# Tencent/FeatherCNN

Measured on AMD Instinct MI355X. Metric: images/sec fp32 forward @224x224, higher is better.
Workload: dtype f32; 1 GPU; vgg16 whole net (40 layers in the model file, 20 after fusion level 3), batch 32 per GPU, 224x224x3, fp32, synthetic ...; net=vgg16, mode=net, per_gpu_batch=32, global_batch=32, parallelism=batch-shard x1, launch=hipGraph replay per step, conv_routing=fhip_conv_select_algo_tuned

## Files before the change

__graft_entry__.py:

```python
from __future__ import annotations

import os
import subprocess
import sys

ROOT = os.path.dirname(os.path.abspath(__file__))
if ROOT not in sys.path:
    sys.path.insert(0, ROOT)


def build() -> None:
    jobs = str(min(8, os.cpu_count() or 1))
    subprocess.run(["make", "-s", "-j", jobs, "-C", os.path.join(ROOT, "feathercnn_amd", "csrc")], check=True)
    subprocess.run(["make", "-s", "-C", os.path.join(ROOT, "oracle"), "port"], check=True)
    subprocess.run(["make", "-s", "-C", os.path.join(ROOT, "oracle"), "ref"], check=True)
    import feathercnn_amd
    feathercnn_amd.load_library()
    from feathercnn_amd import _lib
    _lib.load_gconv_library()
    _lib.load_deconv_library()
    _lib.load_inorm_library()
    _lib.load_shuffle_library()
    _lib.load_canvas_library()
    _lib.load_atrous_library()
    _lib.load_gate_library()
    from feathercnn_amd import provenance
    provenance.write_stamp()


def smoke() -> None:
    import numpy as np
    import torch

    import oracle
    from feathercnn_amd import ConvLayer, ConvParam
    from oracle import conv_geom, nerr, synth

    if not torch.cuda.is_available():
        raise RuntimeError("smoke() needs a GPU")
    if not os.path.exists(os.path.join(ROOT, "feathercnn_amd", "libfeather_hip.so")):
# ... 123 lines not shown
    print(f"smoke tiny_dilated ({sum(a == 'ATROUS' for _, _, a in net.layers())} dilated layers): normalised error = {e:.2e}")
    if not (e <= 1e-4):
        raise AssertionError(f"smoke tiny_dilated: parity failed ({e})")
    import gate_ref
    p, b, i, o = model_zoo.tiny_se()
    x = np.random.default_rng(11).uniform(-1, 1, (2, 3, 24, 24)).astype(np.float32)
    net = Net(fusion=2)
    net.LoadParam(p)
    net.LoadWeights(b)
    net.FeedInput(i, x)
    net.Forward()
    e = gate_ref.nerr(net.Extract(o), gate_ref.Net(p, b).run(i, x, o))
    print(f"smoke tiny_se ({sum(a == 'GATE' and t == 'Pooling' for t, _, a in net.layers())} collapsed SE blocks): normalised error = {e:.2e}")
    if not (e <= 1e-4):
        raise AssertionError(f"smoke tiny_se: parity failed ({e})")
    print("smoke OK")


if __name__ == "__main__":
    build()
    if len(sys.argv) > 1 and sys.argv[1] == "smoke":
        smoke()
```

feathercnn_amd/_lib.py:

```python
from __future__ import annotations

import ctypes
import os

_HERE = os.path.dirname(os.path.abspath(__file__))
_LOADED = {}

STAGE_NAMES = ("wino_input", "wino_gemm", "wino_output", "igemm", "depthwise", "init", "wino_chain")


class fhip_conv_param(ctypes.Structure):
    _fields_ = [(n, ctypes.c_int) for n in (
        "output_channels", "input_channels", "input_h", "input_w", "kernel_h", "kernel_w", "output_h", "output_w",
        "stride_h", "stride_w", "pad_left", "pad_bottom", "pad_right", "pad_top", "group", "bias_term", "activation")]


class fhip_winograd_plan(ctypes.Structure):
    _fields_ = [("tiles_x", ctypes.c_int), ("tiles_y", ctypes.c_int), ("tiles_per_image", ctypes.c_int),
                ("columns", ctypes.c_int), ("columns_padded", ctypes.c_int), ("column_block", ctypes.c_int), ("frequency_points", ctypes.c_int), ("tile_outputs", ctypes.c_int),
                ("in_channels_padded", ctypes.c_int),
                ("out_channels_padded", ctypes.c_int), ("v_offset_bytes", ctypes.c_size_t), ("v_bytes", ctypes.c_size_t),
                ("m_offset_bytes", ctypes.c_size_t), ("m_bytes", ctypes.c_size_t), ("u_bytes", ctypes.c_size_t)]


# ... 23 lines not shown
    "fhip_conv_init": (_I, [_P, _I, _V, _V, _V]),
    "fhip_conv_forward": (_I, [_P, _I, _I, _V, _V, _V, _V, _V, _V]),
    "fhip_winograd_f63_plan": (_I, [_P, _I, ctypes.POINTER(fhip_winograd_plan)]),
    "fhip_winograd_f63_plan_canvas": (_I, [_P, _I, _I, ctypes.POINTER(fhip_winograd_plan)]),
    "fhip_winograd_f63_canvas_param": (_I, [_P, _I, _P]),
    "fhip_winograd_f63_transform_kernel": (_I, [_P, _V, _V, _V]),
    "fhip_winograd_f63_input_transform": (_I, [_P, _I, _V, _V, _V]),
    "fhip_winograd_f63_tile_gemm": (_I, [_P, _I, _V, _V, _V, _V]),
    "fhip_winograd_f63_output_transform": (_I, [_P, _I, _V, _V, _V, _V]),
    "fhip_stage_timing_enable": (_I, [_I]),
    "fhip_stage_timing_collect": (_I, [ctypes.POINTER(ctypes.c_double), ctypes.POINTER(ctypes.c_longlong)]),
    "fhip_last_error": (ctypes.c_char_p, []),
    "fhip_version": (ctypes.c_char_p, []),
    "fhip_device_info": (_I, [ctypes.c_char_p, _I, ctypes.POINTER(_I), ctypes.POINTER(_I)]),
    "fhip_conv_streams_1x1": (_I, [_P, _I, _I]),
    "fhip_calibrate_mfma_f32": (_I, [ctypes.POINTER(ctypes.c_double), ctypes.POINTER(ctypes.c_double), _V]),
    "fhip_relu": (_I, [_V, _V, _SZ, _V]),
    "fhip_add": (_I, [_V, _V, _V, _SZ, _I, _V]),
    "fhip_affine": (_I, [_V, _V, _V, _V, _I, _I, _I, _I, _V]),
    "fhip_conv_can_fuse_residual": (_I, [_P, _I]),
    "fhip_conv_forward_residual": (_I, [_P, _I, _I, _V, _V, _V, _V, _V, _V, _V]),
    "fhip_conv_can_fuse_dw_pw": (_I, [_P, _P, _I]),
    "fhip_conv_forward_dw_pw": (_I, [_P, _P, _I, _V, _V, _V, _V, _V, _V, _V]),
    "fhip_conv_can_chain_winograd": (_I, [_P, _I, _P, _I, _I]),
    "fhip_conv_forward_chained": (_I, [_P, _I, _V, _V, _V, _V, _V, _V, _P, _V, _I, _V]),
    "fhip_winograd_f63_output_to_next_input": (_I, [_P, _P, _I, _V, _V, _V, _I, _V]),
    "fhip_conv_can_fuse_siblings": (_I, [_P, _I, _P, _I, _I]),
    "fhip_conv_siblings_geometry": (_I, [_P, _P, _P]),
    "fhip_conv_forward_siblings": (_I, [_P, _P, _I, _V, _V, _V, _V, _V, _V]),
    "fhip_conv_can_fuse_first_winograd": (_I, [_P, _P, _I, _I]),
# ... 23 lines not shown
    "fhip_net_load_weights_mem": (_I, [_V, _V, _SZ]),
    "fhip_net_load_weights_device": (_I, [_V, _V, _SZ]),
    "fhip_net_feed_input": (_I, [_V, ctypes.c_char_p, _I, _I, _I, _I, _V, _I]),
    "fhip_net_feed_pixels": (_I, [_V, ctypes.c_char_p, _I, _V, _I, _I, _I, _I, _I, _V, _V, _I]),
    "fhip_net_feed_yuv420sp": (_I, [_V, ctypes.c_char_p, _I, _V, _I, _I, _I, _I, _I, _I, _V, _V, _I]),
    "fhip_net_feed_pixel_images": (_I, [_V, ctypes.c_char_p, _I, _V, _I, _I, _I, _V, _V, _I]),
    "fhip_net_forward": (_I, [_V]),
    "fhip_net_extract": (_I, [_V, ctypes.c_char_p, ctypes.POINTER(_V), _PI, _PI, _PI, _PI]),
    "fhip_net_extract_host": (_I, [_V, ctypes.c_char_p, _V, _SZ]),
    "fhip_net_layer_count": (_I, [_V]),
    "fhip_net_layer_info": (_I, [_V, _I, ctypes.c_char_p, ctypes.c_char_p, _I, _PI]),
    "fhip_net_layer_conv_param": (_I, [_V, _I, _P, _PI]),
    "fhip_net_layer_fused_pointwise": (_I, [_V, _I, _P, _PI]),
    "fhip_net_layer_chain": (_I, [_V, _I, _PI, _PI]),
    "fhip_net_layer_canvas": (_I, [_V, _I, _PI]),
    "fhip_net_layer_sibling": (_I, [_V, _I, _PI]),
    "fhip_net_layer_residual": (_I, [_V, _I, _PI]),
    "fhip_net_forward_timed": (_I, [_V, ctypes.POINTER(ctypes.c_float)]),
    "fhip_net_memory": (_I, [_V, ctypes.POINTER(_SZ), ctypes.POINTER(_SZ), ctypes.POINTER(_SZ)]),
}

PIXOUT_SIGNATURES = {
    "fhip_pixout_channels": (_I, [_I]),
    "fhip_float_to_pixels": (_I, [_V, _SZ, _V, _I, _I, _I, _I, _I, _I, _V, _V, _V]),
    "fhip_float_to_pixels_host": (_I, [_V, _SZ, _V, _I, _I, _I, _I, _I, _I, _V, _V, _V]),
    "fhip_pixout_last_error": (ctypes.c_char_p, []),
}

GCONV_SIGNATURES = {
    "fhip_gconv_supported": (_I, [_P]),
# ... 70 lines not shown
    "fhip_atrous_get_buffer_size_route": (_I, [_AP, _I, ctypes.c_char_p, ctypes.POINTER(_SZ), ctypes.POINTER(_SZ)]),
    "fhip_atrous_init_route": (_I, [_AP, _V, _V, _V, ctypes.c_char_p]),
    "fhip_atrous_forward_route": (_I, [_AP, _I, _V, _V, _V, _V, _V, _V, ctypes.c_char_p]),
    "fhip_atrous_last_error": (ctypes.c_char_p, []),
}

GATE_SIGNATURES = {
    "fhip_channel_gate_forward": (_I, [_I, _I, _I, _I, _V, _V, _V, _V, _I, _V]),
    "fhip_squeeze_get_buffer_size": (_I, [_I, _I, _I, _I, ctypes.POINTER(_SZ)]),
    "fhip_squeeze_forward": (_I, [_I, _I, _I, _I, _V, _V, _V, _V]),
    "fhip_excite_forward": (_I, [_I, _I, _I, _V, _V, _V, _V, _V, _V, _I, _I, _FL, _FL, _V]),
    "fhip_excite_forward_slices": (_I, [_I, _I, _I, _I, _V, _V, _V, _V, _V, _V, _I, _I, _FL, _FL, _V]),
    "fhip_gate_activation_forward": (_I, [_I, _V, _V, _I, _I, _I, _FL, _FL, _V]),
    "fhip_gate_route": (_I, [_I, _I, _I, _I, _I, _V, _V, _V, ctypes.c_char_p, _I]),
    "fhip_gate_last_error": (ctypes.c_char_p, []),
}


def _load(path, signatures):
    lib = _LOADED.get(path)
    if lib is None:
        import torch
        if not os.path.exists(path):
            raise RuntimeError(f"feathercnn_amd: HIP library {path} is missing -- run `python -c 'import __graft_entry__ as g; "
                               "g.build()'` (or `make -C feathercnn_amd/csrc`). There is no CPU fallback.")
        lib = ctypes.CDLL(path)
        for name, (res, args) in signatures.items():
            fn = getattr(lib, name)
            fn.restype = res
            fn.argtypes = args
# ... 59 lines not shown

def atrous_path() -> str:
    return os.path.join(_HERE, "libfeather_atrous.so")


def load_atrous_library():
    return _load(atrous_path(), ATROUS_SIGNATURES)


def gate_path() -> str:
    return os.path.join(_HERE, "libfeather_gate.so")


def load_gate_library():
    return _load(gate_path(), GATE_SIGNATURES)
```

feathercnn_amd/csrc/capi.hip:

```cpp
#include <string.h>
#include <stdlib.h>

#include <algorithm>
#include <mutex>
#include <string>
#include <vector>

#include "common.h"
#include "feather_hip/feather_net.h"

namespace fhip
{
int winograd_plan(const fhip_conv_param& p, int batch, fhip_winograd_plan* plan);
int winograd_transform_kernel(const fhip_conv_param& p, float* u, const float* kernel, hipStream_t s);
int winograd_input_transform(const fhip_conv_param& p, int batch, float* v, const float* input, hipStream_t s);
int winograd_tile_gemm(const fhip_conv_param& p, int batch, float* m, const float* u, const float* v, hipStream_t s);
int winograd_output_transform(const fhip_conv_param& p, int batch, float* output, const float* m, const float* bias,
                              hipStream_t s, int pool = 0);
bool winograd_can_pool(const fhip_conv_param& p);
bool winograd_can_chain(const fhip_conv_param& p, const fhip_conv_param& next, int pool);
bool winograd_can_fuse_first(const fhip_conv_param& first, const fhip_conv_param& next, int batch);
fhip_conv_param igemm_twin_geometry(const fhip_conv_param& a, const fhip_conv_param& b);
bool igemm_twin_applicable(const fhip_conv_param& a, const fhip_conv_param& b, int batch);
int igemm_twin_forward(const fhip_conv_param& a, const fhip_conv_param& b, int batch, float* out_a, float* out_b, const float* in, const float* packed,
                       const float* bias, hipStream_t s);
int winograd_input_from_first(const fhip_conv_param& first, const fhip_conv_param& next, int batch, float* v, const float* input,
                              const float* first_kernel, const float* first_bias, hipStream_t s);
int winograd_output_to_next_input(const fhip_conv_param& p, const fhip_conv_param& next, int batch, float* vn, const float* m, const float* bias,
                                  hipStream_t s, int pool);
void igemm_packed_dims(const fhip_conv_param& p, int* kd_padded, int* k_padded);
int igemm_init(const fhip_conv_param& p, float* packed, const float* kernel, hipStream_t s);
int igemm_forward(const fhip_conv_param& p, int batch, float* out, const float* in, const float* packed, const float* bias,
                  float* buffer, bool force_no_act, hipStream_t s, const float* residual = nullptr);
size_t igemm_buffer_bytes(const fhip_conv_param& p, int batch);
size_t igemm_packed_floats(const fhip_conv_param& p);
bool igemm_streams(const fhip_conv_param& p, int batch);
int depthwise_forward(const fhip_conv_param& p, int batch, float* out, const float* in, const float* kernel, const float* bias,
                      hipStream_t s);
int depthwise_init(const fhip_conv_param& p, float* packed, const float* kernel, hipStream_t s);
size_t depthwise_packed_floats(const fhip_conv_param& p, size_t* w12_offset);
bool dwpw_applicable(const fhip_conv_param& dw, const fhip_conv_param& pw, int batch);
int dwpw_forward(const fhip_conv_param& dw, const fhip_conv_param& pw, int batch, float* out, const float* in, const float* dw_packed,
                 const float* dw_bias, const float* pw_packed, const float* pw_bias, hipStream_t s);

static thread_local std::string g_last_error;

int fail(int code, const char* msg)
{
    g_last_error = msg ? msg : "";
    return code;
}
// ... 222 lines not shown
    return conv_forward_impl(p, algo, batch, pooled_output, input, packed, buffer, bias, stream, 1);
}

int fhip_conv_forward_residual(const fhip_conv_param* p, int algo, int batch, float* output, const float* input, const float* packed,
                               float* buffer, const float* bias, const float* residual, void* stream)
{
    if (!residual) return fail(FHIP_E_BADARG, "null residual");
    return conv_forward_impl(p, algo, batch, output, input, packed, buffer, bias, stream, 0, residual);
}

int fhip_conv_streams_1x1(const fhip_conv_param* p, int algo, int batch)
{
    return valid_param(p) && (algo == FHIP_IM2COL || algo == FHIP_NAIVE) && batch >= 1 && igemm_streams(*p, batch) ? 1 : 0;
}

int fhip_conv_can_fuse_residual(const fhip_conv_param* p, int algo) { return valid_param(p) && algo == FHIP_IM2COL ? 1 : 0; }

int fhip_conv_can_fuse_maxpool2(const fhip_conv_param* p, int algo)
{
    return valid_param(p) && algo == FHIP_WINOGRADF63 && winograd_can_pool(*p) ? 1 : 0;
}

int fhip_conv_can_fuse_dw_pw(const fhip_conv_param* dw, const fhip_conv_param* pw, int batch)
{
    return valid_param(dw) && valid_param(pw) && dwpw_applicable(*dw, *pw, batch) ? 1 : 0;
}

int fhip_conv_forward_dw_pw(const fhip_conv_param* dw, const fhip_conv_param* pw, int batch, float* output, const float* input,
                            const float* dw_packed, const float* dw_bias, const float* pw_packed, const float* pw_bias, void* stream)
{
// ... 292 lines not shown
```

feathercnn_amd/csrc/implicit_gemm.hip:

```cpp
#include <string.h>

#include <algorithm>
#include <mutex>

#include "gemm_core.h"
#include "conv_gemm_policy.h"
#include "dwpw_band.h"
#include "stream_gemm.h"
#include "ip_stream.h"

namespace fhip
{

size_t depthwise_packed_floats(const fhip_conv_param& p, size_t* w12_offset);

using ConvShapeBig = GemmShape<128, 64, 16, 2, 2>;
using ConvShapeSmallM = GemmShape<64, 128, 16, 1, 4>;

static bool conv_small_m(int K) { return K <= 64; }
using ConvShapeNarrow = GemmShape<64, 32, 16, 2, 1, 8>;
static bool conv_narrow_n(long long ntot) { return ntot <= 32; }

static bool stream_eligible(const fhip_conv_param& p)
{
// ... 85 lines not shown
    int kdp, kp;
    igemm_packed_dims(p, &kdp, &kp);
    const int m_tiles = kp / 128, n_tiles = (int)((ntot + 63) / 64), kt = kdp / kConvKTile, cus = device_compute_units();
    const long long tiles = (long long)m_tiles * n_tiles;
    if (tiles < cus || tiles > 8LL * cus || (cus & 7)) return 0;
    const int rem = (int)(tiles % cus);
    if (rem == 0 || rem % m_tiles || (m_tiles * (n_tiles - rem / m_tiles)) % 8) return 0;
    int s = std::min(8, cus / rem);
    while (s > 1 && (kt / s < 4 || (rem * s) % 8)) --s;
    if (s < 2) return 0;
    *pieces = s;
    return n_tiles - rem / m_tiles;
}

bool igemm_streams(const fhip_conv_param& p, int batch) { return stream_profitable(p, batch); }

size_t igemm_buffer_bytes(const fhip_conv_param& p, int batch)
{
    if (ip_profitable(p, batch))
        return (ip_xq_floats(p) + (size_t)ip_pieces(p) * p.output_channels * batch) * sizeof(float);
    const int s = igemm_split(p, batch);
    if (s <= 1)
    {
        int pieces;
        const int nt0 = igemm_tail(p, batch, &pieces);
        if (!nt0) return 0;
        const long long tail_cols = ((igemm_columns(p, batch) + 63) / 64 - nt0) * 64;
        return (size_t)pieces * p.output_channels * (size_t)tail_cols * sizeof(float);
    }
    return (size_t)s * p.output_channels * (size_t)igemm_columns(p, batch) * sizeof(float);
// ... 731 lines not shown
```

feathercnn_amd/csrc/net.hip:

```cpp
#include <ctype.h>
#include <dlfcn.h>
#include <errno.h>
#include <float.h>
#include <limits.h>
#include <math.h>
#include <stdarg.h>
#include <stdio.h>
#include <stdlib.h>
#include <string.h>

#include <algorithm>
#include <map>
#include <memory>
#include <mutex>
#include <string>
#include <vector>

#include "common.h"
#include "feather_hip/feather_canvas.h"
#include "feather_hip/feather_atrous.h"
#include "feather_hip/feather_deconv.h"
#include "feather_hip/feather_gate.h"
#include "feather_hip/feather_gconv.h"
#include "feather_hip/feather_inorm.h"
#include "feather_hip/feather_net.h"
#include "feather_hip/feather_shuffle.h"

namespace fhip
{
namespace net
{

static int failf(int code, const char* fmt, ...)
{
    char buf[512];
    va_list ap;
// ... 172 lines not shown
};
static const GateApi* gate_api() { return side_api<GateApi>(); }

struct CanvasApi
{
    decltype(&fhip_canvas_output_to_next_input) chain = nullptr;
    decltype(&fhip_canvas_output_transform) output = nullptr;
    decltype(&fhip_canvas_last_error) last_error = nullptr;
    SideLibrary library()
    {
        return {"libfeather_canvas.so", "a chained Winograd run on 2x2 image canvases", "feather_canvas.h",
                {{&chain, "fhip_canvas_output_to_next_input"}, {&output, "fhip_canvas_output_transform"}, {&last_error, "fhip_canvas_last_error"}}};
    }
};
static const CanvasApi* canvas_api() { return side_api<CanvasApi>(); }

struct ParamDict
{
    static const int kMax = 32;
    struct Entry
    {
        bool loaded = false;
        uint32_t bits = 0;
        std::vector<float> array;
    } e[kMax];

    void clear()
    {
        for (auto& x : e) x = Entry();
    }
// ... 268 lines not shown
    virtual int Reshape()
    {
        if (tops.size() != 1 || bottoms.size() != 1) return failf(NET_E_BASE_RESHAPE, "layer %s: base Reshape needs 1 bottom and 1 top", name.c_str());
        return tops[0]->reshape(bottoms[0]->n, bottoms[0]->c, bottoms[0]->h, bottoms[0]->w);
    }
    virtual int Init(hipStream_t) { return 0; }
    virtual int Forward(hipStream_t) = 0;
    virtual int Fuse(Layer*, int ) { return 0; }
    virtual size_t weight_bytes() const { return 0; }
    virtual size_t arena_bytes() const { return 0; }
    virtual int algo() const { return -1; }
    virtual const fhip_conv_param* conv_param() const { return nullptr; }
    virtual const fhip_conv_param* fused_pointwise(int*) const { return nullptr; }
    virtual void chain_state(int* v_from_previous, int* writes_next_v) const { *v_from_previous = *writes_next_v = 0; }
    virtual int canvas_state() const { return 0; }
    virtual int sibling_state() const { return 0; }
    virtual int residual_state() const { return 0; }
};

static bool is_plain_relu(const Layer* l);

struct Net
{
    std::vector<std::unique_ptr<Layer>> layers;
    std::map<std::string, std::unique_ptr<Blob>> blobs;
    std::vector<std::unique_ptr<Blob>> shadowed;
    hipStream_t stream = nullptr;
    int fusion = 1;
    bool use_graph = false;
    bool tuned_selection = false;
// ... 457 lines not shown
    {
        *v_from_previous = head ? 2 : chain_in ? 1 : 0;
        *writes_next_v = head_of ? 2 : chain_next ? 1 : 0;
    }
    int canvas_state() const override { return canvas ? 1 : 0; }
};

struct InnerProductLayer : Layer
{
    fhip_conv_param p;
    size_t input_size = 0, output_size = 0, weight_data_size = 0;
    std::vector<float> w_host, b_host;
    DeviceVec packed, bias;
    size_t buffer_bytes = 0, packed_bytes = 0;
    bool inited = false;

    InnerProductLayer() { memset(&p, 0, sizeof(p)); }
    int LoadParam(const ParamDict& pd) override
    {
        output_size = pd.get(0, 0);
        p.bias_term = pd.get(1, 0);
        weight_data_size = pd.get(2, 0);
        if (pd.get(0, 0) < 1) return failf(NET_E_SHAPE, "layer %s: num_output must be positive", name.c_str());
        if (pd.get(2, 0) < 0 || weight_data_size % output_size)
            return failf(NET_E_SHAPE, "layer %s: weight_data_size is no whole number of rows of num_output", name.c_str());
        input_size = weight_data_size / output_size;
        p.input_channels = (int)input_size;
        p.output_channels = (int)output_size;
        p.input_h = p.input_w = p.kernel_h = p.kernel_w = p.stride_h = p.stride_w = p.group = 1;
        fhip_conv_assign_output_dim(&p);
// ... 26 lines not shown
        if (rc) return rc;
        rc = fhip_conv_init(&p, FHIP_IM2COL, packed.d, raw.d, s);
        if (rc) return rc;
        if (p.bias_term)
        {
            rc = bias.upload(b_host.data(), b_host.size(), s);
            if (rc) return rc;
        }
        FHIP_CHECK_HIP(hipStreamSynchronize(s));
        std::vector<float>().swap(w_host);
        inited = true;
        return 0;
    }
    int Forward(hipStream_t s) override
    {
        return fhip_conv_forward(&p, FHIP_IM2COL, bottoms[0]->n, tops[0]->data, bottoms[0]->data, packed.d, (float*)net->arena.d,
                                 p.bias_term ? bias.d : nullptr, s);
    }
    int Fuse(Layer* next, int) override
    {
        if (is_plain_relu(next))
        {
            p.activation = FHIP_ACT_RELU;
            return 1;
        }
        return 0;
    }
    size_t weight_bytes() const override { return packed.bytes + bias.bytes; }
    size_t arena_bytes() const override { return buffer_bytes; }
    int algo() const override { return FHIP_IM2COL; }
};

struct ReluLayer : Layer
{
    float slope = 0.f;
    int LoadParam(const ParamDict& pd) override
    {
        slope = pd.get(0, 0.f);
        return 0;
    }
    int Reshape() override
    {
        if (slope != 0.f && !inorm_api()) return FHIP_E_UNSUPPORTED;
        return Layer::Reshape();
// ... 1428 lines not shown
        fhip_winograd_plan pl;
        const int rc = fhip_winograd_f63_plan_canvas(&c->p, c->bottoms[0]->n, c->canvas ? 2 : 1, &pl);
        if (rc) return rc;
        c->run_plan = pl;
        slot[c->chain_pos & 1] = std::max(slot[c->chain_pos & 1], up(pl.v_bytes));
        msz = std::max(msz, up(pl.m_bytes));
    }
    net.chain_slot[0] = 0;
    net.chain_slot[1] = slot[0];
    net.chain_m = slot[0] + slot[1];
    for (size_t i = 0; i < L; ++i)
        if (conv[i] && (conv[i]->chain_in || conv[i]->chain_next || conv[i]->head)) conv[i]->chain_bytes = slot[0] + slot[1] + msz;
    return 0;
}

static int plan_siblings(Net& net)
{
    const size_t L = net.layers.size();
    std::vector<ConvLayer*> conv(L, nullptr);
    for (size_t i = 0; i < L; ++i)
        if (net.layers[i]->type == "Convolution")
        {
            conv[i] = static_cast<ConvLayer*>(net.layers[i].get());
            conv[i]->sib = conv[i]->sib_of = nullptr;
        }
    if (net.fusion < 2) return 0;
    auto root = [](const Blob* b) { return b->alias ? b->alias : b; };
    auto plain = [](const ConvLayer* c) {
        return c && !c->pw && !c->residual && !c->fuse_pool && !c->chain_in && !c->chain_next && !c->head && !c->head_of && !c->sib && !c->sib_of &&
               c->algo_ == FHIP_IM2COL && c->tops.size() == 1 && c->bottoms.size() == 1;
// ... 18 lines not shown
}

static int reshape_all(Net& net)
{
    net.drop_graph();
    size_t need = 0;
    for (auto& l : net.layers)
    {
        const int rc = l->Reshape();
        if (rc) return rc;
    }
    {
        int rc = plan_chains(net);
        if (rc) return rc;
        if ((rc = plan_siblings(net))) return rc;
    }
    for (auto& l : net.layers) need = std::max(need, l->arena_bytes());
    if (need > net.arena.bytes)
    {
        const int rc = net.arena.resize(need);
        if (rc) return rc;
    }
    net.shapes_dirty = false;
    return plan_concurrency(net);
}

static int prepare(Net& net)
{
    if (!net.param_loaded) return failf(NET_E_IO, "Network has not been loaded. Please load the param file first.");
    if (!net.weights_loaded)
// ... 628 lines not shown
{
    NET_GUARD(n);
    if (index < 0 || index >= (int)n->impl.layers.size() || !v_from_previous || !writes_next_v) return fail(FHIP_E_BADARG, "layer index out of range");
    n->impl.layers[index]->chain_state(v_from_previous, writes_next_v);
    return FHIP_OK;
}

int fhip_net_layer_canvas(fhip_net* n, int index, int* canvas)
{
    NET_GUARD(n);
    if (index < 0 || index >= (int)n->impl.layers.size() || !canvas) return fail(FHIP_E_BADARG, "layer index out of range");
    *canvas = n->impl.layers[index]->canvas_state();
    return FHIP_OK;
}

int fhip_net_forward_timed(fhip_net* n, float* ms)
{
    NET_GUARD(n);
    if (!ms) return fail(FHIP_E_BADARG, "null argument");
    if (!n->more.empty())
        return fail(FHIP_E_UNSUPPORTED, "per-layer timing of a net with sub-batch replicas: kernels of concurrent replicas share the chip, "
                                        "so their durations are not layer times -- time a net created without fhip_net_set_sub_batches");
    Net& net = n->impl;
    int rc = prepare(net);
    if (rc) return rc;
    const size_t L = net.layers.size();
    std::vector<hipEvent_t> ev(L + 1);
    for (auto& e : ev) FHIP_CHECK_HIP(hipEventCreate(&e));
    FHIP_CHECK_HIP(hipEventRecord(ev[0], net.stream));
    for (size_t i = 0; i < L && rc == 0; ++i)
// ... 36 lines not shown
```

feathercnn_amd/net.py:

```python
from __future__ import annotations

import ctypes

import numpy as np

from . import _lib
from .booster import ALGO_NAMES, FeatherHipError, _check, _stream


ROUTE_GCONV = 100
ROUTE_NAMES = dict(ALGO_NAMES)
ROUTE_NAMES[ROUTE_GCONV] = "GCONV"
ROUTE_DECONV = 101
ROUTE_NAMES[ROUTE_DECONV] = "DECONV"
ROUTE_INORM = 102
ROUTE_NAMES[ROUTE_INORM] = "INORM"
ROUTE_SHUFFLE = 103
ROUTE_NAMES[ROUTE_SHUFFLE] = "SHUFFLE"
ROUTE_ATROUS = 104
ROUTE_NAMES[ROUTE_ATROUS] = "ATROUS"
ROUTE_GATE = 105
ROUTE_NAMES[ROUTE_GATE] = "GATE"

class Net:
# ... 201 lines not shown
            if self._lib.fhip_net_layer_chain(self._h, i, ctypes.byref(a), ctypes.byref(b)) == 0 and (a.value or b.value):
                if raw:
                    out[i] = (a.value, b.value)
                elif a.value == 1 or b.value == 1:
                    out[i] = (a.value == 1, b.value == 1)
        return out

    def canvases(self):
        out = []
        for i in range(self._lib.fhip_net_layer_count(self._h)):
            c = ctypes.c_int()
            if self._lib.fhip_net_layer_canvas(self._h, i, ctypes.byref(c)) == 0 and c.value:
                out.append(i)
        return out

    def forward_timed(self):
        n = self._lib.fhip_net_layer_count(self._h)
        ms = (ctypes.c_float * max(n, 1))()
        _check(self._lib.fhip_net_forward_timed(self._h, ms), "fhip_net_forward_timed")
        info = self.layers()
        return [(t, nm, a, ms[i]) for i, (t, nm, a) in enumerate(info)]

    def memory(self):
        v = [ctypes.c_size_t() for _ in range(3)]
        _check(self._lib.fhip_net_memory(self._h, *[ctypes.byref(x) for x in v]), "fhip_net_memory")
        return {"blob_bytes": v[0].value, "weight_bytes": v[1].value, "arena_bytes": v[2].value}


def _p(t):
    return ctypes.c_void_p(t.data_ptr()) if t is not None else None
# ... 47 lines not shown
```

include/feather_hip/feather_hip.h:

```cpp
#ifndef FEATHER_HIP_H_
#define FEATHER_HIP_H_

#include <stddef.h>

#ifdef __cplusplus
extern "C" {
#endif

#define FHIP_API __attribute__((visibility("default")))

enum fhip_conv_algo
{
    FHIP_NAIVE = 0,
    FHIP_IM2COL = 1,
    FHIP_SGECONV = 2,
    FHIP_DEPTHWISE = 3,
    FHIP_WINOGRADF63 = 4,
    FHIP_WINOGRADF63FUSED = 5,
    FHIP_WINOGRADF23 = 6
};

enum fhip_activation
{
    FHIP_ACT_NONE = 0,
// ... 82 lines not shown
    FHIP_STAGE_WINO_INPUT = 0,
    FHIP_STAGE_WINO_GEMM = 1,
    FHIP_STAGE_WINO_OUTPUT = 2,
    FHIP_STAGE_IGEMM = 3,
    FHIP_STAGE_DEPTHWISE = 4,
    FHIP_STAGE_INIT = 5,
    FHIP_STAGE_WINO_CHAIN = 6,
    FHIP_STAGE_COUNT = 7
};
FHIP_API int fhip_stage_timing_enable(int on);
FHIP_API int fhip_stage_timing_collect(double* ms, long long* launches);

FHIP_API const char* fhip_last_error(void);
FHIP_API const char* fhip_version(void);
FHIP_API int fhip_conv_streams_1x1(const fhip_conv_param* param, int algo, int batch);

FHIP_API int fhip_device_info(char* name, int name_len, int* compute_units, int* lds_bytes);
FHIP_API int fhip_calibrate_mfma_f32(double* tflops, double* shader_mhz, void* stream);

#ifdef __cplusplus
}
#endif
#endif
```

include/feather_hip/feather_net.h:

```cpp
#ifndef FEATHER_NET_H_
#define FEATHER_NET_H_

#include "feather_hip/feather_hip.h"

#ifdef __cplusplus
extern "C" {
#endif


FHIP_API int fhip_relu(float* y, const float* x, size_t count, void* stream);

FHIP_API int fhip_add(float* y, const float* a, const float* b, size_t count, int relu, void* stream);

FHIP_API int fhip_affine(float* y, const float* x, const float* mul, const float* add, int batch, int channels, int hw,
                         int relu, void* stream);


enum
{
    FHIP_PIXEL_CONVERT_SHIFT = 16,
    FHIP_PIXEL_RGB = 1,
    FHIP_PIXEL_BGR = (1 << 1),
    FHIP_PIXEL_GRAY = (1 << 2),
    FHIP_PIXEL_RGBA = (1 << 3),
// ... 101 lines not shown
FHIP_API int fhip_net_extract(fhip_net* net, const char* blob_name, float** device_ptr, int* n, int* c, int* h, int* w);
FHIP_API int fhip_net_extract_host(fhip_net* net, const char* blob_name, float* host, size_t capacity);

FHIP_API int fhip_net_layer_count(fhip_net* net);
#define FHIP_NET_ROUTE_GCONV 100
#define FHIP_NET_ROUTE_DECONV 101
#define FHIP_NET_ROUTE_INORM 102
#define FHIP_NET_ROUTE_SHUFFLE 103
#define FHIP_NET_ROUTE_ATROUS 104
#define FHIP_NET_ROUTE_GATE 105
FHIP_API int fhip_net_layer_info(fhip_net* net, int index, char* type, char* name, int len, int* algo);
FHIP_API int fhip_net_layer_conv_param(fhip_net* net, int index, fhip_conv_param* param, int* batch);
FHIP_API int fhip_net_layer_fused_pointwise(fhip_net* net, int index, fhip_conv_param* param, int* one_kernel);
FHIP_API int fhip_net_layer_chain(fhip_net* net, int index, int* v_from_previous, int* writes_next_v);
FHIP_API int fhip_net_layer_canvas(fhip_net* net, int index, int* canvas);
FHIP_API int fhip_net_layer_sibling(fhip_net* net, int index, int* state);
FHIP_API int fhip_net_layer_residual(fhip_net* net, int index, int* state);
FHIP_API int fhip_net_forward_timed(fhip_net* net, float* ms);
FHIP_API int fhip_net_memory(fhip_net* net, size_t* blob_bytes, size_t* weight_bytes, size_t* arena_bytes);

#ifdef __cplusplus
}
#endif
#endif
```

Measured before the change: 10120 images/s.

## Route chained InnerProduct layers through split-K weight-streaming tail library

After: 10140 images/s, median of 6. Within noise of the previous version (+0.2%).

```diff
diff --git a/__graft_entry__.py b/__graft_entry__.py
--- a/__graft_entry__.py
+++ b/__graft_entry__.py
@@ -24,6 +24,7 @@
     _lib.load_canvas_library()
     _lib.load_atrous_library()
     _lib.load_gate_library()
+    _lib.load_fctail_library()
     from feathercnn_amd import provenance
     provenance.write_stamp()
 
@@ -177,6 +178,14 @@
     print(f"smoke tiny_se ({sum(a == 'GATE' and t == 'Pooling' for t, _, a in net.layers())} collapsed SE blocks): normalised error = {e:.2e}")
     if not (e <= 1e-4):
         raise AssertionError(f"smoke tiny_se: parity failed ({e})")
+    from feathercnn_amd import fctail
+    w, xin = (torch.from_numpy(np.random.default_rng(12).uniform(-1, 1, s).astype(np.float32)).to(dev) for s in ((256, 1024), (2, 1024)))
+    fc = fctail.FcLayer(w, None, relu=True, batch=2)
+    y, _ = fctail.reduce_pack(fc, fctail.stream(fc, fctail.pack_input(xin), 4), 4)
+    e = nerr(y.cpu().numpy(), fc.forward_plain(xin).cpu().numpy())
+    print(f"smoke fctail 1024 -> 256: normalised difference to the plain route = {e:.2e}")
+    if not (e <= 1e-4):
+        raise AssertionError(f"smoke fctail: parity failed ({e})")
     print("smoke OK")
 
 
diff --git a/feathercnn_amd/_lib.py b/feathercnn_amd/_lib.py
--- a/feathercnn_amd/_lib.py
+++ b/feathercnn_amd/_lib.py
@@ -61,6 +61,7 @@
     "fhip_version": (ctypes.c_char_p, []),
     "fhip_device_info": (_I, [ctypes.c_char_p, _I, ctypes.POINTER(_I), ctypes.POINTER(_I)]),
     "fhip_conv_streams_1x1": (_I, [_P, _I, _I]),
+    "fhip_conv_ip_weights": (_I, [_P, _V, ctypes.POINTER(_V), _PI, _PI]),
     "fhip_calibrate_mfma_f32": (_I, [ctypes.POINTER(ctypes.c_double), ctypes.POINTER(ctypes.c_double), _V]),
     "fhip_relu": (_I, [_V, _V, _SZ, _V]),
     "fhip_add": (_I, [_V, _V, _V, _SZ, _I, _V]),
@@ -114,6 +115,7 @@
     "fhip_net_layer_fused_pointwise": (_I, [_V, _I, _P, _PI]),
     "fhip_net_layer_chain": (_I, [_V, _I, _PI, _PI]),
     "fhip_net_layer_canvas": (_I, [_V, _I, _PI]),
+    "fhip_net_layer_fc_tail": (_I, [_V, _I, _PI]),
     "fhip_net_layer_sibling": (_I, [_V, _I, _PI]),
     "fhip_net_layer_residual": (_I, [_V, _I, _PI]),
     "fhip_net_forward_timed": (_I, [_V, ctypes.POINTER(ctypes.c_float)]),
@@ -214,6 +216,16 @@
     "fhip_gate_activation_forward": (_I, [_I, _V, _V, _I, _I, _I, _FL, _FL, _V]),
     "fhip_gate_route": (_I, [_I, _I, _I, _I, _I, _V, _V, _V, ctypes.c_char_p, _I]),
     "fhip_gate_last_error": (ctypes.c_char_p, []),
+}
+
+FCTAIL_SIGNATURES = {
+    "fhip_fctail_supported": (_I, [_I, _I, _I]),
+    "fhip_fctail_pieces": (_I, [_I, _I, _PI]),
+    "fhip_fctail_get_buffer_size": (_I, [_I, _I, _I, _I, ctypes.POINTER(_SZ), ctypes.POINTER(_SZ)]),
+    "fhip_fctail_pack_input": (_I, [_I, _I, _V, _V, _V]),
+    "fhip_fctail_stream": (_I, [_I, _I, _I, _I, _V, _V, _V, _V]),
+    "fhip_fctail_reduce_pack": (_I, [_I, _I, _I, _V, _V, _V, _V, _I, _V]),
+    "fhip_fctail_last_error": (ctypes.c_char_p, []),
 }
 
 
@@ -303,3 +315,11 @@
 
 def load_gate_library():
     return _load(gate_path(), GATE_SIGNATURES)
+
+
+def fctail_path() -> str:
+    return os.path.join(_HERE, "libfeather_fctail.so")
+
+
+def load_fctail_library():
+    return _load(fctail_path(), FCTAIL_SIGNATURES)
diff --git a/feathercnn_amd/csrc/capi.hip b/feathercnn_amd/csrc/capi.hip
--- a/feathercnn_amd/csrc/capi.hip
+++ b/feathercnn_amd/csrc/capi.hip
@@ -35,6 +35,7 @@
 size_t igemm_buffer_bytes(const fhip_conv_param& p, int batch);
 size_t igemm_packed_floats(const fhip_conv_param& p);
 bool igemm_streams(const fhip_conv_param& p, int batch);
+bool igemm_ip_weights(const fhip_conv_param& p, size_t* offset_floats, int* Kg, int* KQ);
 int depthwise_forward(const fhip_conv_param& p, int batch, float* out, const float* in, const float* kernel, const float* bias,
                       hipStream_t s);
 int depthwise_init(const fhip_conv_param& p, float* packed, const float* kernel, hipStream_t s);
@@ -287,6 +288,15 @@
     return valid_param(p) && (algo == FHIP_IM2COL || algo == FHIP_NAIVE) && batch >= 1 && igemm_streams(*p, batch) ? 1 : 0;
 }
 
+int fhip_conv_ip_weights(const fhip_conv_param* p, const float* packed, const float** wp, int* m_groups, int* k_octets)
+{
+    if (!valid_param(p) || !packed || !wp || !m_groups || !k_octets) return fail(FHIP_E_BADARG, "bad argument");
+    size_t off;
+    if (!igemm_ip_weights(*p, &off, m_groups, k_octets)) return fail(FHIP_E_UNSUPPORTED, "this geometry has no streamed InnerProduct weight image");
+    *wp = packed + off;
+    return FHIP_OK;
+}
+
 int fhip_conv_can_fuse_residual(const fhip_conv_param* p, int algo) { return valid_param(p) && algo == FHIP_IM2COL ? 1 : 0; }
 
 int fhip_conv_can_fuse_maxpool2(const fhip_conv_param* p, int algo)
diff --git a/feathercnn_amd/csrc/implicit_gemm.hip b/feathercnn_amd/csrc/implicit_gemm.hip
--- a/feathercnn_amd/csrc/implicit_gemm.hip
+++ b/feathercnn_amd/csrc/implicit_gemm.hip
@@ -123,6 +123,17 @@
 }
 
 bool igemm_streams(const fhip_conv_param& p, int batch) { return stream_profitable(p, batch); }
+
+bool igemm_ip_weights(const fhip_conv_param& p, size_t* offset_floats, int* Kg, int* KQ)
+{
+    if (!ip_eligible(p)) return false;
+    int kdp, kp;
+    igemm_packed_dims(p, &kdp, &kp);
+    *offset_floats = (size_t)kdp * kp + (stream_eligible(p) ? (size_t)p.output_channels * p.input_channels : 0);
+    *Kg = ip_kg(p);
+    *KQ = ip_kq(p);
+    return true;
+}
 
 size_t igemm_buffer_bytes(const fhip_conv_param& p, int batch)
 {
diff --git a/feathercnn_amd/csrc/net.hip b/feathercnn_amd/csrc/net.hip
--- a/feathercnn_amd/csrc/net.hip
+++ b/feathercnn_amd/csrc/net.hip
@@ -20,6 +20,7 @@
 #include "feather_hip/feather_canvas.h"
 #include "feather_hip/feather_atrous.h"
 #include "feather_hip/feather_deconv.h"
+#include "feather_hip/feather_fctail.h"
 #include "feather_hip/feather_gate.h"
 #include "feather_hip/feather_gconv.h"
 #include "feather_hip/feather_inorm.h"
@@ -222,6 +223,29 @@
     }
 };
 static const CanvasApi* canvas_api() { return side_api<CanvasApi>(); }
+
+struct FctailApi
+{
+    decltype(&fhip_fctail_supported) supported = nullptr;
+    decltype(&fhip_fctail_pieces) pieces = nullptr;
+    decltype(&fhip_fctail_get_buffer_size) get_buffer_size = nullptr;
+    decltype(&fhip_fctail_pack_input) pack_input = nullptr;
+    decltype(&fhip_fctail_stream) stream = nullptr;
+    decltype(&fhip_fctail_reduce_pack) reduce_pack = nullptr;
+    decltype(&fhip_fctail_last_error) last_error = nullptr;
+    SideLibrary library()
+    {
+        return {"libfeather_fctail.so", "a run of InnerProduct layers at a batch of at most 32", "feather_fctail.h",
+                {{&supported, "fhip_fctail_supported"}, {&pieces, "fhip_fctail_pieces"}, {&get_buffer_size, "fhip_fctail_get_buffer_size"},
+                 {&pack_input, "fhip_fctail_pack_input"}, {&stream, "fhip_fctail_stream"}, {&reduce_pack, "fhip_fctail_reduce_pack"},
+                 {&last_error, "fhip_fctail_last_error"}}};
+    }
+};
+static const FctailApi* fctail_api() { return side_api<FctailApi>(); }
+
+#ifndef FHIP_FCTAIL_PARTS
+#define FHIP_FCTAIL_PARTS 2
+#endif
 
 struct ParamDict
 {
@@ -520,6 +544,7 @@
     virtual const fhip_conv_param* fused_pointwise(int*) const { return nullptr; }
     virtual void chain_state(int* v_from_previous, int* writes_next_v) const { *v_from_previous = *writes_next_v = 0; }
     virtual int canvas_state() const { return 0; }
+    virtual int fc_tail_state() const { return 0; }
     virtual int sibling_state() const { return 0; }
     virtual int residual_state() const { return 0; }
 };
@@ -1007,6 +1032,10 @@
     DeviceVec packed, bias;
     size_t buffer_bytes = 0, packed_bytes = 0;
     bool inited = false;
+    int tail_pos = -1, tail_pieces = 0;
+    bool tail_fed = false;
+    InnerProductLayer* tail_feeds = nullptr;
+    size_t tail_xq_off = 0, tail_partial_off = 0, tail_bytes = 0;
 
     InnerProductLayer() { memset(&p, 0, sizeof(p)); }
     int LoadParam(const ParamDict& pd) override
@@ -1063,9 +1092,30 @@
     }
     int Forward(hipStream_t s) override
     {
+        if (tail_pos >= 0) return forward_tail(s);
         return fhip_conv_forward(&p, FHIP_IM2COL, bottoms[0]->n, tops[0]->data, bottoms[0]->data, packed.d, (float*)net->arena.d,
                                  p.bias_term ? bias.d : nullptr, s);
     }
+    int forward_tail(hipStream_t s)
+    {
+        const FctailApi* api = fctail_api();
+        if (!api) return FHIP_E_UNSUPPORTED;
+        const float* wp = nullptr;
+        int kg = 0, kq = 0;
+        int rc = fhip_conv_ip_weights(&p, packed.d, &wp, &kg, &kq);
+        if (rc) return rc;
+        char* base = reinterpret_cast<char*>(net->arena.d);
+        float *xq = reinterpret_cast<float*>(base + tail_xq_off), *partial = reinterpret_cast<float*>(base + tail_partial_off);
+        const int n = bottoms[0]->n, C = p.input_channels, K = p.output_channels, relu = p.activation == FHIP_ACT_RELU ? 1 : 0;
+        const float* b = p.bias_term ? bias.d : nullptr;
+        if (!tail_fed) rc = api->pack_input(C, n, xq, bottoms[0]->data, s);
+        if (!rc) rc = api->stream(C, K, n, tail_pieces, partial, wp, xq, s);
+        if (!rc)
+            rc = api->reduce_pack(K, n, tail_pieces, tops[0]->data, tail_feeds ? reinterpret_cast<float*>(base + tail_feeds->tail_xq_off) : nullptr,
+                                  partial, b, relu, s);
+        return rc ? failf(rc, "layer %s: %s", name.c_str(), api->last_error()) : 0;
+    }
+    int fc_tail_state() const override { return tail_pos < 0 ? 0 : tail_fed ? 2 : 1; }
     int Fuse(Layer* next, int) override
     {
         if (is_plain_relu(next))
@@ -1076,7 +1126,7 @@
         return 0;
     }
     size_t weight_bytes() const override { return packed.bytes + bias.bytes; }
-    size_t arena_bytes() const override { return buffer_bytes; }
+    size_t arena_bytes() const override { return std::max(buffer_bytes, tail_bytes); }
     int algo() const override { return FHIP_IM2COL; }
 };
 
@@ -2535,6 +2585,86 @@
     return 0;
 }
 
+static int plan_fc_tails(Net& net)
+{
+    const size_t L = net.layers.size();
+    for (auto& l : net.layers)
+        if (l->type == "InnerProduct")
+        {
+            InnerProductLayer* ip = static_cast<InnerProductLayer*>(l.get());
+            ip->tail_pos = -1;
+            ip->tail_fed = false;
+            ip->tail_feeds = nullptr;
+            ip->tail_bytes = 0;
+        }
+    if (net.fusion < 3 || !(FHIP_FCTAIL_PARTS & 2)) return 0;
+    auto root = [](const Blob* b) {
+        while (b->alias) b = b->alias;
+        return b;
+    };
+    auto passes = [](const Layer* l) { return l->type == "Dropout" && static_cast<const DropoutLayer*>(l)->scale == 1.f; };
+    auto member = [](Layer* l) -> InnerProductLayer* {
+        if (l->type != "InnerProduct" || l->bottoms.size() != 1 || l->tops.size() != 1) return nullptr;
+        InnerProductLayer* ip = static_cast<InnerProductLayer*>(l);
+        const int n = ip->bottoms[0]->n;
+        if (ip->tail_pos >= 0 || ip->p.input_channels < 1024 || ip->p.output_channels < 256 || n < 1 || n > 32) return nullptr;
+        if (ip->p.activation != FHIP_ACT_NONE && ip->p.activation != FHIP_ACT_RELU) return nullptr;
+        return ip;
+    };
+    auto readers = [&](const Blob* top) {
+        std::vector<Layer*> r;
+        for (auto& l : net.layers)
+            for (Blob* b : l->bottoms)
+                if (root(b) == root(top) && !passes(l.get())) r.push_back(l.get());
+        return r;
+    };
+    auto up = [](size_t x) { return (x + 255) / 256 * 256; };
+    const FctailApi* api = nullptr;
+    for (size_t i = 0; i < L; ++i)
+    {
+        InnerProductLayer* first = member(net.layers[i].get());
+        if (!first) continue;
+        std::vector<InnerProductLayer*> run{first};
+        for (;;)
+        {
+            const std::vector<Layer*> r = readers(run.back()->tops[0]);
+            InnerProductLayer* nx = r.size() == 1 ? member(r[0]) : nullptr;
+            if (!nx || std::find(run.begin(), run.end(), nx) != run.end()) break;
+            run.push_back(nx);
+        }
+        if (run.size() < 2) continue;
+        if (!api && !(api = fctail_api())) return FHIP_E_UNSUPPORTED;
+        size_t xq[2] = {0, 0}, part = 0;
+        for (size_t k = 0; k < run.size(); ++k)
+        {
+            InnerProductLayer* ip = run[k];
+            const int n = ip->bottoms[0]->n, C = ip->p.input_channels, K = ip->p.output_channels;
+            if (!api->supported(C, K, n))
+                return failf(FHIP_E_UNSUPPORTED, "layer %s: libfeather_fctail.so refuses a geometry the plain streaming route takes", ip->name.c_str());
+            int rc = api->pieces(C, K, &ip->tail_pieces);
+            size_t xb = 0, pb = 0;
+            if (!rc) rc = api->get_buffer_size(C, K, n, ip->tail_pieces, &xb, &pb);
+            if (rc) return failf(rc, "layer %s: %s", ip->name.c_str(), api->last_error());
+            xq[k & 1] = std::max(xq[k & 1], up(xb));
+            part = std::max(part, up(pb));
+        }
+        for (size_t k = 0; k < run.size(); ++k)
+        {
+            InnerProductLayer* ip = run[k];
+            ip->tail_pos = (int)k;
+            ip->tail_xq_off = (k & 1) ? xq[0] : 0;
+            ip->tail_partial_off = xq[0] + xq[1];
+            ip->tail_bytes = xq[0] + xq[1] + part;
+            if (k + 1 < run.size())
+            {
+                ip->tail_feeds = run[k + 1];
+                run[k + 1]->tail_fed = true;
+            }
+        }
+    }
+    return 0;
+}
+
 static int plan_siblings(Net& net)
 {
     const size_t L = net.layers.size();
@@ -2583,6 +2713,7 @@
         int rc = plan_chains(net);
         if (rc) return rc;
         if ((rc = plan_siblings(net))) return rc;
+        if ((rc = plan_fc_tails(net))) return rc;
     }
     for (auto& l : net.layers) need = std::max(need, l->arena_bytes());
     if (need > net.arena.bytes)
@@ -3241,6 +3372,14 @@
     return FHIP_OK;
 }
 
+int fhip_net_layer_fc_tail(fhip_net* n, int index, int* state)
+{
+    NET_GUARD(n);
+    if (index < 0 || index >= (int)n->impl.layers.size() || !state) return fail(FHIP_E_BADARG, "layer index out of range");
+    *state = n->impl.layers[index]->fc_tail_state();
+    return FHIP_OK;
+}
+
 int fhip_net_forward_timed(fhip_net* n, float* ms)
 {
     NET_GUARD(n);
diff --git a/feathercnn_amd/csrc_fctail/fctail.hip b/feathercnn_amd/csrc_fctail/fctail.hip
--- /dev/null
+++ b/feathercnn_amd/csrc_fctail/fctail.hip
@@ -0,0 +1,146 @@
+#include <hip/hip_runtime.h>
+#include <stdint.h>
+
+#include <algorithm>
+#include <string>
+
+#include "feather_hip/feather_fctail.h"
+#include "ip_stream.h"
+
+namespace fhip
+{
+
+static thread_local std::string g_error;
+
+int fail(int code, const char* msg)
+{
+    g_error = msg;
+    return code;
+}
+int fail_hip(hipError_t e, const char* what)
+{
+    g_error = std::string(what) + ": " + hipGetErrorString(e);
+    return FHIP_E_HIP;
+}
+int device_compute_units()
+{
+    static thread_local int dev_cached = -1, cus_cached = 0;
+    int dev = 0;
+    if (hipGetDevice(&dev) != hipSuccess) return 256;
+    if (dev != dev_cached)
+    {
+        int cus = 0;
+        if (hipDeviceGetAttribute(&cus, hipDeviceAttributeMultiprocessorCount, dev) != hipSuccess || cus < 1) cus = 256;
+        cus_cached = cus;
+        dev_cached = dev;
+    }
+    return cus_cached;
+}
+
+__device__ __forceinline__ float fc_sum_pieces(const float* __restrict__ src, size_t stride, int S, const float* __restrict__ bias, int m, int has_bias,
+                                               int relu)
+{
+    float acc = 0.f;
+    int s = 0;
+    for (; s + 4 <= S; s += 4)
+    {
+        const float v0 = src[(size_t)s * stride], v1 = src[(size_t)(s + 1) * stride], v2 = src[(size_t)(s + 2) * stride], v3 = src[(size_t)(s + 3) * stride];
+        acc = (((acc + v0) + v1) + v2) + v3;
+    }
+    for (; s < S; ++s) acc += src[(size_t)s * stride];
+    if (has_bias) acc += bias[m];
+    if (relu) acc = fmaxf(acc, 0.f);
+    return acc;
+}
+
+__global__ __launch_bounds__(256) void fc_reduce_pack_kernel(float* __restrict__ out, float* __restrict__ xq, const float* __restrict__ partial,
+                                                             const float* __restrict__ bias, int K, int batch, int S, int has_bias, int relu)
+{
+    __shared__ float t[8][33];
+    const int q = blockIdx.x, ml = threadIdx.x >> 5, n = threadIdx.x & 31, m = 8 * q + ml;
+    float v = 0.f;
+    if (n < batch && m < K) v = fc_sum_pieces(partial + (size_t)m * batch + n, (size_t)K * batch, S, bias, m, has_bias, relu);
+    t[ml][n] = v;
+    __syncthreads();
+    {
+        const int on = threadIdx.x >> 3, om = threadIdx.x & 7;
+        if (on < batch && 8 * q + om < K) out[(size_t)on * K + 8 * q + om] = t[om][on];
+    }
+    if (xq && threadIdx.x < 64)
+    {
+        const int lane = threadIdx.x, xn = lane & 31, h = lane >> 5;
+        reinterpret_cast<float4*>(xq)[(size_t)q * 64 + lane] = make_float4(t[h][xn], t[2 + h][xn], t[4 + h][xn], t[6 + h][xn]);
+    }
+}
+
+static bool aligned16(const void* p) { return (reinterpret_cast<uintptr_t>(p) & 15) == 0; }
+static bool supported(int C, int K, int batch) { return C >= 1024 && K >= 256 && batch >= 1 && batch <= 32; }
+static int max_pieces(int C) { return std::max(1, ceil_div(C, 8) / 8); }
+
+static int pieces_of(int C, int K)
+{
+    const int want = device_compute_units() * 3 / std::max(1, ceil_div(ceil_div(K, 32), 4));
+    return std::max(1, std::min(want, max_pieces(C)));
+}
+
+}
+
+using namespace fhip;
+
+extern "C"
+{
+
+int fhip_fctail_supported(int C, int K, int batch) { return supported(C, K, batch) ? 1 : 0; }
+
+int fhip_fctail_pieces(int C, int K, int* pieces)
+{
+    if (!pieces) return fail(FHIP_E_BADARG, "bad argument");
+    if (!supported(C, K, 1)) return fail(FHIP_E_UNSUPPORTED, "the weight-streaming InnerProduct takes C >= 1024 and K >= 256");
+    *pieces = pieces_of(C, K);
+    return FHIP_OK;
+}
+
+int fhip_fctail_get_buffer_size(int C, int K, int batch, int pieces, size_t* xq_bytes, size_t* partial_bytes)
+{
+    if (!xq_bytes || !partial_bytes || pieces < 1 || batch < 1 || batch > 32) return fail(FHIP_E_BADARG, "bad argument");
+    if (!supported(C, K, batch)) return fail(FHIP_E_UNSUPPORTED, "the weight-streaming InnerProduct takes C >= 1024 and K >= 256");
+    *xq_bytes = (size_t)ceil_div(C, 8) * 256 * sizeof(float);
+    *partial_bytes = (size_t)pieces * batch * K * sizeof(float);
+    return FHIP_OK;
+}
+
+int fhip_fctail_pack_input(int C, int batch, float* xq, const float* x, void* stream)
+{
+    if (!xq || !x || !aligned16(xq) || !aligned16(x) || batch < 1 || batch > 32 || C < 1) return fail(FHIP_E_BADARG, "bad argument");
+    const int KQ = ceil_div(C, 8);
+    hipLaunchKernelGGL(ip_pack_input_kernel, dim3(ceil_div(KQ, kIpPackOctets)), dim3(256), 0, (hipStream_t)stream, xq, x, batch, C, KQ);
+    FHIP_CHECK_HIP(hipGetLastError());
+    return FHIP_OK;
+}
+
+int fhip_fctail_stream(int C, int K, int batch, int pieces, float* partial, const float* wp, const float* xq, void* stream)
+{
+    if (!partial || !wp || !xq || !aligned16(partial) || !aligned16(wp) || !aligned16(xq)) return fail(FHIP_E_BADARG, "bad argument");
+    if (batch < 1 || batch > 32) return fail(FHIP_E_BADARG, "bad argument");
+    if (!supported(C, K, batch)) return fail(FHIP_E_UNSUPPORTED, "the weight-streaming InnerProduct takes C >= 1024 and K >= 256");
+    if (pieces < 1 || pieces > max_pieces(C)) return fail(FHIP_E_BADARG, "bad argument: a piece is at least 8 k-octets long");
+    IpStreamParams q;
+    q.wp = wp, q.xq = xq, q.partial = partial, q.K = K, q.Kg = ceil_div(K, 32), q.KQ = ceil_div(C, 8), q.S = pieces, q.batch = batch;
+    hipLaunchKernelGGL(ip_stream_kernel<4>, dim3((unsigned)pieces * (unsigned)ceil_div(q.Kg, 4)), dim3(256), 0, (hipStream_t)stream, q);
+    FHIP_CHECK_HIP(hipGetLastError());
+    return FHIP_OK;
+}
+
+int fhip_fctail_reduce_pack(int K, int batch, int pieces, float* out, float* xq_next, const float* partial, const float* bias, int relu, void* stream)
+{
+    if (!out || !partial || !aligned16(out) || !aligned16(partial) || !aligned16(xq_next)) return fail(FHIP_E_BADARG, "bad argument");
+    if (K < 1 || batch < 1 || batch > 32 || pieces < 1) return fail(FHIP_E_BADARG, "bad argument");
+    hipLaunchKernelGGL(fc_reduce_pack_kernel, dim3(ceil_div(K, 8)), dim3(256), 0, (hipStream_t)stream, out, xq_next, partial, bias, K, batch, pieces,
+                       bias ? 1 : 0, relu ? 1 : 0);
+    FHIP_CHECK_HIP(hipGetLastError());
+    return FHIP_OK;
+}
+
+const char* fhip_fctail_last_error(void) { return fhip::g_error.c_str(); }
+
+}
diff --git a/feathercnn_amd/fctail.py b/feathercnn_amd/fctail.py
--- /dev/null
+++ b/feathercnn_amd/fctail.py
@@ -0,0 +1,83 @@
+from __future__ import annotations
+
+import ctypes
+
+from . import _lib
+from .booster import IM2COL, ConvLayer, ConvParam, FeatherHipError, _check, _ptr, _stream
+
+
+def _check_fctail(rc, what):
+    if rc != 0:
+        raise FeatherHipError(f"{what} failed ({rc}): {_lib.load_fctail_library().fhip_fctail_last_error().decode()}")
+
+
+def pieces(C: int, K: int) -> int:
+    s = ctypes.c_int()
+    _check_fctail(_lib.load_fctail_library().fhip_fctail_pieces(C, K, ctypes.byref(s)), "fhip_fctail_pieces")
+    return s.value
+
+
+def buffer_floats(C: int, K: int, batch: int, npieces: int):
+    a, b = ctypes.c_size_t(), ctypes.c_size_t()
+    _check_fctail(_lib.load_fctail_library().fhip_fctail_get_buffer_size(C, K, batch, npieces, ctypes.byref(a), ctypes.byref(b)),
+                  "fhip_fctail_get_buffer_size")
+    return a.value // 4, b.value // 4
+
+
+class FcLayer:
+
+    def __init__(self, weight, bias=None, relu=False, batch=1):
+        K, C = weight.shape
+        self.C, self.K, self.batch, self.relu, self.bias = C, K, batch, bool(relu), bias
+        self.param = ConvParam.make(C, K, 1, k=1, s=1, p=0, bias=bias is not None, act=1 if relu else 0, batch=batch)
+        self.plain = ConvLayer(self.param, weight.reshape(K, C, 1, 1).contiguous(), bias, algo=IM2COL)
+        wp, kg, kq = ctypes.c_void_p(), ctypes.c_int(), ctypes.c_int()
+        c = self.param._c()
+        _check(_lib.load_library().fhip_conv_ip_weights(ctypes.byref(c), _ptr(self.plain.packed), ctypes.byref(wp), ctypes.byref(kg), ctypes.byref(kq)),
+               "fhip_conv_ip_weights")
+        off = (wp.value - self.plain.packed.data_ptr()) // 4
+        self.Kg, self.KQ = kg.value, kq.value
+        self.wp = self.plain.packed[off:off + self.Kg * self.KQ * 256]
+
+    def forward_plain(self, x, fill=None):
+        import torch
+        out = torch.empty((self.batch, self.K, 1, 1), dtype=torch.float32, device=x.device)
+        scratch = torch.empty(max(self.plain.buffer_bytes // 4, 1), dtype=torch.float32, device=x.device)
+        if fill is not None:
+            out.fill_(fill), scratch.fill_(fill)
+        return self.plain.Forward(x.reshape(self.batch, self.C, 1, 1), out, scratch).reshape(self.batch, self.K)
+
+
+def pack_input(x, fill=None):
+    import torch
+    batch, C = x.shape
+    xq = torch.empty((C + 7) // 8 * 256, dtype=torch.float32, device=x.device)
+    if fill is not None:
+        xq.fill_(fill)
+    _check_fctail(_lib.load_fctail_library().fhip_fctail_pack_input(C, batch, _ptr(xq), _ptr(x), _stream()), "fhip_fctail_pack_input")
+    return xq
+
+
+def stream(layer: FcLayer, xq, npieces=None, fill=None):
+    import torch
+    npieces = pieces(layer.C, layer.K) if npieces is None else npieces
+    _, pf = buffer_floats(layer.C, layer.K, layer.batch, max(npieces, 1))
+    partial = torch.empty(pf, dtype=torch.float32, device=xq.device)
+    if fill is not None:
+        partial.fill_(fill)
+    _check_fctail(_lib.load_fctail_library().fhip_fctail_stream(layer.C, layer.K, layer.batch, npieces, _ptr(partial), _ptr(layer.wp), _ptr(xq), _stream()),
+                  "fhip_fctail_stream")
+    return partial
+
+
+def reduce_pack(layer: FcLayer, partial, npieces, hand_over=True, fill=None):
+    import torch
+    out = torch.empty((layer.batch, layer.K), dtype=torch.float32, device=partial.device)
+    xq = torch.empty((layer.K + 7) // 8 * 256, dtype=torch.float32, device=partial.device) if hand_over else None
+    if fill is not None:
+        out.fill_(fill)
+        if xq is not None:
+            xq.fill_(fill)
+    _check_fctail(_lib.load_fctail_library().fhip_fctail_reduce_pack(layer.K, layer.batch, npieces, _ptr(out), _ptr(xq), _ptr(partial), _ptr(layer.bias),
+                                                                     int(layer.relu), _stream()), "fhip_fctail_reduce_pack")
+    return out, xq
diff --git a/feathercnn_amd/net.py b/feathercnn_amd/net.py
--- a/feathercnn_amd/net.py
+++ b/feathercnn_amd/net.py
@@ -239,6 +239,14 @@
                 out.append(i)
         return out
 
+    def fc_tails(self):
+        out = {}
+        for i in range(self._lib.fhip_net_layer_count(self._h)):
+            st = ctypes.c_int()
+            if self._lib.fhip_net_layer_fc_tail(self._h, i, ctypes.byref(st)) == 0 and st.value:
+                out[i] = st.value
+        return out
+
     def forward_timed(self):
         n = self._lib.fhip_net_layer_count(self._h)
         ms = (ctypes.c_float * max(n, 1))()
diff --git a/include/feather_hip/feather_fctail.h b/include/feather_hip/feather_fctail.h
--- /dev/null
+++ b/include/feather_hip/feather_fctail.h
@@ -0,0 +1,32 @@
+#ifndef FEATHER_HIP_FEATHER_FCTAIL_H_
+#define FEATHER_HIP_FEATHER_FCTAIL_H_
+
+#include <stddef.h>
+
+#ifdef __cplusplus
+extern "C"
+{
+#endif
+
+#define FHIP_FCTAIL_API __attribute__((visibility("default")))
+
+FHIP_FCTAIL_API int fhip_fctail_supported(int C, int K, int batch);
+
+FHIP_FCTAIL_API int fhip_fctail_pieces(int C, int K, int* pieces);
+
+FHIP_FCTAIL_API int fhip_fctail_get_buffer_size(int C, int K, int batch, int pieces, size_t* xq_bytes, size_t* partial_bytes);
+
+FHIP_FCTAIL_API int fhip_fctail_pack_input(int C, int batch, float* xq, const float* x, void* stream);
+
+FHIP_FCTAIL_API int fhip_fctail_stream(int C, int K, int batch, int pieces, float* partial, const float* wp, const float* xq, void* stream);
+
+FHIP_FCTAIL_API int fhip_fctail_reduce_pack(int K, int batch, int pieces, float* out, float* xq_next, const float* partial, const float* bias,
+                                            int relu, void* stream);
+
+FHIP_FCTAIL_API const char* fhip_fctail_last_error(void);
+
+#ifdef __cplusplus
+}
+#endif
+
+#endif
diff --git a/include/feather_hip/feather_hip.h b/include/feather_hip/feather_hip.h
--- a/include/feather_hip/feather_hip.h
+++ b/include/feather_hip/feather_hip.h
@@ -120,6 +120,7 @@
 FHIP_API const char* fhip_last_error(void);
 FHIP_API const char* fhip_version(void);
 FHIP_API int fhip_conv_streams_1x1(const fhip_conv_param* param, int algo, int batch);
+FHIP_API int fhip_conv_ip_weights(const fhip_conv_param* param, const float* packed, const float** wp, int* m_groups, int* k_octets);
 
 FHIP_API int fhip_device_info(char* name, int name_len, int* compute_units, int* lds_bytes);
 FHIP_API int fhip_calibrate_mfma_f32(double* tflops, double* shader_mhz, void* stream);
diff --git a/include/feather_hip/feather_net.h b/include/feather_hip/feather_net.h
--- a/include/feather_hip/feather_net.h
+++ b/include/feather_hip/feather_net.h
@@ -139,6 +139,7 @@
 FHIP_API int fhip_net_layer_fused_pointwise(fhip_net* net, int index, fhip_conv_param* param, int* one_kernel);
 FHIP_API int fhip_net_layer_chain(fhip_net* net, int index, int* v_from_previous, int* writes_next_v);
 FHIP_API int fhip_net_layer_canvas(fhip_net* net, int index, int* canvas);
+FHIP_API int fhip_net_layer_fc_tail(fhip_net* net, int index, int* state);
 FHIP_API int fhip_net_layer_sibling(fhip_net* net, int index, int* state);
 FHIP_API int fhip_net_layer_residual(fhip_net* net, int index, int* state);
 FHIP_API int fhip_net_forward_timed(fhip_net* net, float* ms);
```
